# qdrant/quantization

Measured on AMD Instinct MI355X. Metric: scored vectors/sec, 10Mx768 u8 dot, higher is better.
Workload: dtype u8; 1 GPU; 10000000 x 768 store: f32 U[0,1) -> scalar u8 (dot); per step: encode_query + score_all over the shard; quantizer=u8, rows_per_gpu=10000000, dim=768, distance=dot, exchange=scores, gather_group=1, launch=single rank, world_size_seen=1, encode_ahead=False, total_rows=10000000, queries=16

## Files before the change

quantization_amd/csrc/common.hpp:

```cpp
#pragma once

#include <hip/hip_runtime.h>

#include <algorithm>
#include <atomic>
#include <mutex>
#include <cstdarg>
#include <cstdint>
#include <cstdlib>
#include <cstdio>
#include <cstring>
#include <string>
#include <vector>

#include "json.hpp"

#include "../../include/quantization_amd.h"

namespace qamd {

std::string &last_error();
qamd_status fail(qamd_status st, const char *fmt, ...) __attribute__((format(printf, 2, 3)));

#define QAMD_HIP(expr)                                                                      \
// ... 35 lines not shown
    return getenv(name);
#else
    (void)name;
    return nullptr;
#endif
}
inline uint64_t dev_env_u64(const char *name, uint64_t dflt) {
    const char *e = dev_env(name);
    if (!e || !*e) return dflt;
    char *end = nullptr;
    const unsigned long long v = strtoull(e, &end, 10);
    return (*end == 0 && v > 0) ? (uint64_t)v : dflt;
}
inline uint64_t stage_bytes(uint64_t dflt) {
    static const uint64_t v = dev_env_u64("QAMD_DEV_STAGE_BYTES", 0);
    return v ? v : dflt;
}
inline bool host_whole_allowed() {
    static const bool on = [] { const char *e = dev_env("QAMD_DEV_HOST_WHOLE"); return !(e && e[0] == '0'); }();
    return on;
}
inline bool u8_packed_allowed() {
    static const bool on = [] { const char *e = dev_env("QAMD_DEV_U8_PACKED"); return !(e && e[0] == '0'); }();
    return on;
}
inline uint64_t pq_planar_max_rows() {
    static const uint64_t v = dev_env_u64("QAMD_DEV_PQ_PLANAR_ROWS", 1ull << 28);
    return v;
}
inline uint64_t pq_skew_max_rows() {
    static const uint64_t v = dev_env_u64("QAMD_DEV_PQ_SKEW_ROWS", 1ull << 30);
    return v;
}

class DeviceOnce {
  public:
    template <class F> qamd_status run(F &&setup) {
        int dev = 0;
        if (hipGetDevice(&dev) != hipSuccess || dev < 0 || dev > 63) return setup();
        const uint64_t bit = 1ull << dev;
        if (done_.load(std::memory_order_acquire) & bit) return QAMD_OK;
        std::lock_guard<std::mutex> g(mu_);
        if (done_.load(std::memory_order_relaxed) & bit) return QAMD_OK;
        const qamd_status st = setup();
        if (st == QAMD_OK) done_.fetch_or(bit, std::memory_order_release);
        return st;
// ... 137 lines not shown
```

quantization_amd/csrc/u8.hip:

```cpp
#include <algorithm>
#include <cmath>
#include <cstdlib>
#include <memory>
#include <type_traits>
#include <vector>

#include "common.hpp"
#include "lists.hpp"
#include "multi_reduce.hpp"
#include "topk.hpp"
#include "topk_device.hpp"
#include "rescore.hpp"
#include "u8_internal.hpp"

#pragma clang fp contract(off)

using namespace qamd;

namespace {

constexpr int kBlock = 256;
constexpr int kScanBlock = 512;
constexpr uint64_t kRowPad = 1024;
constexpr uint64_t kQuantileSample = 100000;
// ... 149 lines not shown
        uint32_t acc = 0;
#pragma unroll
        for (int it = 0; it < ITERS; it++) acc = IS_L1 ? sad16(v[u][it], q[it], acc) : dot16(v[u][it], q[it], acc);
        acc = group_sum<G>(acc);
        if (sub == (u % G)) mine = epilogue(multiplier, acc, q_off, v_off[u / G], 0.0f, EPI_POINT);
        if ((u % G) == G - 1 || u == UNROLL - 1) {
            constexpr int dummy = 0;
            (void)dummy;
            const int first = (u / G) * G;
            const uint64_t row = base + (uint64_t)(first + sub) * RW + rslot;
            if (sub <= u - first && row < n_rows) {
                if (FILTER) topk_offer(filt, pivot, mine, (uint32_t)row);
                else __builtin_nontemporal_store(mine, out + row);
            }
        }
    }
}

constexpr uint32_t kPackBlockRows = 64;
constexpr uint32_t kPackBlockChunk = kPackBlockRows;

__device__ __forceinline__ uint4 and16(const uint4 &v, uint32_t m) { return make_uint4(v.x & m, v.y & m, v.z & m, v.w & m); }

template <bool FILTER>
__global__ __launch_bounds__(kScanBlock) __attribute__((amdgpu_waves_per_eu(8, 8))) void u8_scan_blocked_kernel(
    const uint4 *__restrict__ image, const float *__restrict__ offsets, const uint4 *__restrict__ qcodes,
    const float *__restrict__ q_off_p, float multiplier, uint32_t n_rows, uint32_t pchunks, uint32_t n_extra,
    uint32_t split, float *__restrict__ out, TopkFilter filt) {
    __shared__ uint32_t partial[kScanBlock];
    const uint32_t lane = threadIdx.x & 63;
    const uint32_t wave = __builtin_amdgcn_readfirstlane(threadIdx.x >> 6);
    const uint32_t part = wave & (split - 1);
    const uint64_t block = (uint64_t)blockIdx.x * ((kScanBlock / 64) / split) + wave / split;
    const uint64_t row = block * kPackBlockRows + lane;
    const bool live = block * kPackBlockRows < n_rows;
    const uint32_t n_rest = pchunks - 7 * n_extra, n_groups = n_extra + (n_rest ? 1 : 0);
    const uint32_t g_begin = live ? n_groups * part / split : 0, g_end = live ? n_groups * (part + 1) / split : 0;
    const uint4 *blk = image + block * pchunks * kPackBlockChunk;
    const uint32_t lane16 = lane * 16;
    auto chunk_ptr = [&](uint32_t c) {
        return reinterpret_cast<const uint4 *>(reinterpret_cast<const char *>(blk + (uint64_t)c * kPackBlockChunk) + lane16);
    };
    const uint32_t gf_end = g_end < n_extra ? g_end : n_extra;
    const bool has_rest = g_end > n_extra;

    uint4 v[7];
    uint32_t acc = 0;
    auto eat = [&](uint32_t g, auto refill) {
        const uint4 *q = qcodes + 7 * g;
        const uint4 qx = qcodes[pchunks + g];
#pragma unroll
        for (int i = 0; i < 7; i++) {
            const uint4 w = v[i];
            acc = dot16(and16(w, 0x7F7F7F7Fu), q[i], acc) + (dot16(and16(w, 0x80808080u), qx, 0) >> (7 - i));
            if (decltype(refill)::value) {
                __builtin_amdgcn_sched_barrier(0);
                v[i] = ld_nt(chunk_ptr(7 * (g + 1) + i));
                __builtin_amdgcn_sched_barrier(0);
            }
        }
    };
    if (g_begin < gf_end) {
#pragma unroll
        for (int i = 0; i < 7; i++) v[i] = ld_nt(chunk_ptr(7 * g_begin + i));
    }
    const float v_off = offsets[row];
    const float q_off = *q_off_p;
    uint32_t pivot = 0;
    if (FILTER) pivot = *filt.pivot_key;
    if (g_begin < gf_end) {
        for (uint32_t g = g_begin; g + 1 < gf_end; g++) eat(g, std::true_type{});
        eat(gf_end - 1, std::false_type{});
    }
    if (has_rest) {
        const uint4 *q = qcodes + 7 * n_extra;
#pragma unroll
        for (int i = 0; i < 7; i++)
            if ((uint32_t)i < n_rest) v[i] = ld_nt(chunk_ptr(7 * n_extra + i));
#pragma unroll
        for (int i = 0; i < 7; i++)
            if ((uint32_t)i < n_rest) acc = dot16(and16(v[i], 0x7F7F7F7Fu), q[i], acc);
    }
    if (split > 1) {
        partial[threadIdx.x] = acc;
        __syncthreads();
        if (part == 0)
            for (uint32_t p = 1; p < split; p++) acc += partial[threadIdx.x + 64 * p];
    }
    if (part == 0 && row < n_rows) {
        const float score = epilogue(multiplier, acc, q_off, v_off, 0.0f, EPI_POINT);
        if (FILTER) topk_offer(filt, pivot, score, (uint32_t)row);
        else __builtin_nontemporal_store(score, out + row);
    }
}

template <int G, int ITERS, int UNROLL, int NQ, bool IS_L1, bool EXACT, bool FILTER>
__global__ __launch_bounds__(kScanBlock) void u8_scan_multi_kernel(
    const uint4 *__restrict__ codes, const float *__restrict__ offsets, const uint8_t *__restrict__ qcodes,
    uint32_t q_pitch, const float *__restrict__ q_offs, uint32_t nq_valid ,
    float multiplier, uint32_t n_rows, uint32_t row_chunks, float *__restrict__ out ,
    uint64_t out_pitch, TopkFilterSlices slices) {
    static_assert(G >= NQ, "one lane of the row group per query");
    constexpr int RW = 64 / G;
    constexpr int TILE = RW * UNROLL;
    constexpr int TPW = NQ;
    const int lane = threadIdx.x & 63;
    const int sub = lane % G, rslot = lane / G;
    const uint64_t wave = ((uint64_t)blockIdx.x * kScanBlock + threadIdx.x) >> 6;
    if (wave * TILE * TPW >= n_rows) return;
    uint4 q[NQ][ITERS];
#pragma unroll
    for (int j = 0; j < NQ; j++) {
        const uint4 *qj = reinterpret_cast<const uint4 *>(qcodes + (size_t)((uint32_t)j < nq_valid ? j : nq_valid - 1) * q_pitch);
#pragma unroll
        for (int it = 0; it < ITERS; it++) {
// ... 782 lines not shown
            else QAMD_U8_GO(false, false);
        }
#undef QAMD_U8_GO
    }
};

uint32_t blocked_split(uint64_t count) {
    const uint64_t blocks = (count + kPackBlockRows - 1) / kPackBlockRows;
    const uint64_t want = (uint64_t)device_info().cu_count * 16;
    uint32_t split = 1;
    while (split < 8 && blocks * split < want) split *= 2;
    return split;
}

void launch_scan_blocked(const qamd_u8 *h, const uint4 *qc, const float *qo, float *out, const TopkFilter *filt,
                         hipStream_t s) {
    const uint32_t split = blocked_split(h->count), blocks_per_wg = (kScanBlock / 64) / split;
    const uint64_t blocks = (h->count + kPackBlockRows - 1) / kPackBlockRows;
    const unsigned grid = (unsigned)((blocks + blocks_per_wg - 1) / blocks_per_wg);
    h->last_scan_split.store((int)split, std::memory_order_relaxed);
#define QAMD_U8_BLOCKED(FI)                                                                                          \
    hipLaunchKernelGGL((u8_scan_blocked_kernel<FI>), dim3(grid), dim3(kScanBlock), 0, s, h->packed.as<uint4>(),       \
                       h->offsets.as<float>(), qc, qo, h->meta.multiplier, (uint32_t)h->count, h->packed_chunks,      \
                       h->row_chunks - h->packed_chunks, split, out, filt ? *filt : TopkFilter{})
    if (filt) QAMD_U8_BLOCKED(true);
    else QAMD_U8_BLOCKED(false);
#undef QAMD_U8_BLOCKED
}

template <bool IS_L1>
bool launch_scan(const qamd_u8 *h, const uint4 *qc, const float *qo, float *out, const TopkFilter *filt,
                 hipStream_t s) {
    using L = ScanLaunch<IS_L1>;
    const bool packed = !IS_L1 && h->packed_chunks != 0;
    h->last_scan_packed.store(packed ? 1 : 0, std::memory_order_relaxed);
    if (packed) return launch_scan_blocked(h, qc, qo, out, filt, s), true;
    const uint32_t rc = h->row_chunks;
    if (rc == 1) return L::template go<1, 1, 4>(h, qc, qo, out, filt, s), true;
    if (rc == 2) return L::template go<2, 1, 4>(h, qc, qo, out, filt, s), true;
    if (rc <= 4) return L::template go<4, 1, 8>(h, qc, qo, out, filt, s), true;
    if (rc <= 8) return L::template go<8, 1, 8>(h, qc, qo, out, filt, s), true;
    switch ((rc + 15) / 16) {
        case 1: return L::template go<16, 1, 8>(h, qc, qo, out, filt, s), true;
        case 2: return L::template go<16, 2, 4>(h, qc, qo, out, filt, s), true;
        case 3: return L::template go<16, 3, 4>(h, qc, qo, out, filt, s), true;
        case 4: return L::template go<16, 4, 2>(h, qc, qo, out, filt, s), true;
        case 5: return L::template go<16, 5, 2>(h, qc, qo, out, filt, s), true;
        case 6: return L::template go<16, 6, 2>(h, qc, qo, out, filt, s), true;
        case 7: return L::template go<16, 7, 2>(h, qc, qo, out, filt, s), true;
        case 8: return L::template go<16, 8, 2>(h, qc, qo, out, filt, s), true;
// ... 90 lines not shown
    } else {
        if (exact) QAMD_U8_MULTI(true, false);
        else QAMD_U8_MULTI(false, false);
    }
#undef QAMD_U8_MULTI
}

bool lane_order(const qamd_u8 *h) {
    return h->lane_mode == 1 && h->meta.vector_parameters.distance_type != QAMD_L1;
}

uint32_t multi_width(const qamd_u8 *h) {
    const uint32_t rc = h->row_chunks, iters = (rc + 15) / 16;
    const bool l1 = h->meta.vector_parameters.distance_type == QAMD_L1;
    if (rc < 9 || iters > 8 || lane_order(h)) return 0;
    return l1 && iters <= 3 ? 8 : iters <= 6 ? 4 : 2;
}

template <bool IS_L1>
bool launch_multi(const qamd_u8 *h, uint32_t nq_valid, const uint8_t *qcodes, uint64_t q_pitch, const float *q_offs,
                  float *out, const TopkFilterSlices *slices, hipStream_t s) {
    const uint32_t iters = (h->row_chunks + 15) / 16, width = multi_width(h);
    if (nq_valid < 2 || nq_valid > width) return false;
#define QAMD_U8_MULTI_IT(IT, UN)                                                                              \
    case IT:                                                                                                  \
        if constexpr (IS_L1 && IT <= 3) {                                                                     \
            if (nq_valid > 4) {                                                                               \
                launch_multi_shape<IS_L1, 16, IT, UN, 8>(h, qcodes, q_pitch, q_offs, nq_valid, out, slices, s); \
                return true;                                                                                  \
            }                                                                                                 \
        }                                                                                                     \
        if (nq_valid > 2) launch_multi_shape<IS_L1, 16, IT, UN, (IT <= 6 ? 4 : 2)>(h, qcodes, q_pitch, q_offs, nq_valid, out, slices, s); \
        else launch_multi_shape<IS_L1, 16, IT, UN, 2>(h, qcodes, q_pitch, q_offs, nq_valid, out, slices, s);  \
        return true;
    switch (iters) {
        QAMD_U8_MULTI_IT(1, 4) QAMD_U8_MULTI_IT(2, 2) QAMD_U8_MULTI_IT(3, 2) QAMD_U8_MULTI_IT(4, 2)
        QAMD_U8_MULTI_IT(5, 1) QAMD_U8_MULTI_IT(6, 1) QAMD_U8_MULTI_IT(7, 1) QAMD_U8_MULTI_IT(8, 1)
        default: break;
    }
#undef QAMD_U8_MULTI_IT
    return false;
}

bool fused_capable(const qamd_u8 *h) { return !lane_order(h) && h->row_chunks <= 128; }

bool u8_small_plan(const qamd_u8 *h, uint32_t k, SmallTopkPlan &plan) {
// ... 1112 lines not shown
```

quantization_amd/csrc/u8_batch.hip:

```cpp
#include <algorithm>
#include <cmath>
#include <cstdlib>
#include <memory>
#include <mutex>
#include <type_traits>
#include <vector>

#include "common.hpp"
#include "topk.hpp"
#include "topk_device.hpp"
#include "rescore.hpp"
#include "u8_internal.hpp"
#include "batch_common.hpp"
#include "u8_gemm_route.hpp"

#pragma clang fp contract(off)

using namespace qamd;

namespace {

constexpr int TQ = 256;
#ifdef QAMD_DEV
__device__ unsigned long long *g_gemm_stamps = nullptr;
// ... 486 lines not shown
                            }
                        }
                    }
                }
            }
        }
        if (ti < 3) stamp(4 + 3 * (int)ti);
        if (g == 1 && ti + 1 < my_tiles) PP_BARRIER();
    }
    stamp(15);
    if (stamps) stamps[14] = dbg_flagged;
    if (stamps) stamps[13] = __builtin_amdgcn_s_getreg((31 << 11) | 4);
    if (MODE != 0 && lane == 0) filt.wave_counts[filt.wave_base + blockIdx.x * 8 + wave] = *wcount_s;
}

template <int MI> struct RsShape {
    static constexpr int MJ = 2;
    static constexpr int TQ = 32 * MI;
    static constexpr int CHUNK = 32 * MJ;
    static constexpr int TR = 8 * CHUNK;
    static constexpr int KB = 128;
    static constexpr size_t CONSTS = 3 * 128 * sizeof(float) + 64;
    static constexpr size_t SLOTS = 8 * 4096;
    static size_t lds_bytes(uint32_t ad) { return (size_t)TQ * (round_up((uint64_t)ad, KB) + 16) + CONSTS + SLOTS; }
};

template <int MODE, bool LOW, int MI, bool NT>
__global__ __launch_bounds__(512) void u8_gemm_rs_kernel(const uint8_t *__restrict__ codes,
                                                        const float *__restrict__ v_offsets,
                                                        const uint8_t *__restrict__ qcodes, uint32_t q_pitch,
                                                        const float *__restrict__ q_offsets, float multiplier,
                                                        uint32_t n_rows, uint32_t n_queries, uint32_t ad,
                                                        uint32_t q_tiles, uint32_t row_lanes,
                                                        float *__restrict__ out, uint64_t out_pitch,
                                                        BatchFilter filt) {
    extern __shared__ __attribute__((aligned(1024))) uint8_t lds_raw[];
    using Shape = RsShape<MI>;
    constexpr int MJ = Shape::MJ, TQ = Shape::TQ, CHUNK = Shape::CHUNK, TR = Shape::TR, KB = Shape::KB;
    const int t = threadIdx.x, lane = t & 63;
    const int wave = __builtin_amdgcn_readfirstlane(t >> 6);
    const int r = lane & 31, h = lane >> 5;
    const uint32_t b = blockIdx.x, xcd = b & 7u, j = b >> 3;
    if (j >= row_lanes * q_tiles) return;
    const uint32_t q_tile = j % q_tiles, row_lane = j / q_tiles;
    const uint32_t q0 = q_tile * TQ;
    const uint32_t nkb = __builtin_amdgcn_readfirstlane((ad + KB - 1) / KB);
    const uint32_t PA = nkb * KB + 16;
    const uint32_t n_rtiles = (n_rows + TR - 1) / TR;
    const uint32_t first = xcd + 8 * row_lane, step = 8 * row_lanes;
    const uint32_t my_tiles =
        __builtin_amdgcn_readfirstlane(first < n_rtiles ? (n_rtiles - first + step - 1) / step : 0u);

    float *q_off_s = reinterpret_cast<float *>(lds_raw + (size_t)TQ * PA);
    float *pivot_s = q_off_s + 128;
    int *bq_s = reinterpret_cast<int *>(pivot_s + 128);
    uint32_t *wcount_s = reinterpret_cast<uint32_t *>(bq_s + 128) + wave;
    constexpr bool LARGEST = MODE == 1;
    if (MODE != 0 && lane == 0) *wcount_s = 0;
    if (t < TQ) {
        const float qo = q_offsets[q0 + t];
        q_off_s[t] = qo;
        if (MODE != 0) {
            const float pv = filt.pivot_scores[q0 + t];
            pivot_s[t] = pv;
            bq_s[t] = pp_query_bound<LOW>(pv, qo, multiplier, q0 + t < n_queries);
        }
    }
    {
        const uint32_t per_row = nkb * (KB / 16);
        for (uint32_t idx = t; idx < (uint32_t)TQ * per_row; idx += 512) {
            const uint32_t row = idx / per_row, k = (idx % per_row) * 16;
            v4i v = {0, 0, 0, 0};
            if (k < q_pitch) v = *reinterpret_cast<const v4i *>(qcodes + (uint64_t)(q0 + row) * q_pitch + k);
            *reinterpret_cast<v4i *>(lds_raw + row * PA + k) = v;
        }
    }
    __syncthreads();
    if (my_tiles == 0) {
        if (MODE != 0 && lane == 0) filt.wave_counts[filt.wave_base + blockIdx.x * 8 + wave] = 0;
        return;
    }

    const uint64_t row_bytes = ad;
    const uint32_t l8 = (uint32_t)lane & 7u, lrow = (uint32_t)lane >> 3;
    const uint8_t *pf0 = codes + ((uint64_t)first * TR + wave * CHUNK + lrow) * row_bytes + 16 * l8;
    const uint64_t i_stride = (uint64_t)8 * row_bytes;
    const uint64_t wrap_advance = (uint64_t)step * TR * row_bytes - (uint64_t)nkb * KB;
    uint32_t pf_kb = 0, pf_left = my_tiles * nkb - 1;
    v4i L[8];
    auto prefetch = [&]() {
        if (NT) {
#pragma unroll
            for (int i = 0; i < 8; i++) L[i] = __builtin_nontemporal_load(reinterpret_cast<const v4i *>(pf0 + i * i_stride));
        } else {
#pragma unroll
            for (int i = 0; i < 8; i++) L[i] = *reinterpret_cast<const v4i *>(pf0 + i * i_stride);
        }
        uint64_t adv = KB;
        if (++pf_kb == nkb) {
            pf_kb = 0;
            adv += wrap_advance;
        }
        if (pf_left == 0) {
            adv = 0;
            pf_kb = 0;
        } else {
            pf_left--;
        }
        pf0 += adv;
    };
    uint8_t *slot = lds_raw + (size_t)TQ * PA + Shape::CONSTS + (size_t)wave * 4096;
    uint8_t *wr = slot + lrow * 128 + ((l8 ^ (lrow & 7u)) * 16);
    const uint32_t rbase = (uint32_t)r * 128u + (((4u * (uint32_t)h) ^ ((uint32_t)r & 4u)) * 16u);
    const uint8_t *rd = slot + rbase;
    const uint32_t r3 = (uint32_t)r & 3u;
    v4i F[MJ][4];
    auto transpose = [&]() {
#pragma unroll
        for (int jj = 0; jj < MJ; jj++) {
#pragma unroll
            for (int i = 0; i < 4; i++) *reinterpret_cast<v4i *>(wr + 1024 * i) = L[4 * jj + i];
#pragma unroll
            for (int x = 0; x < 4; x++) F[jj][x] = *reinterpret_cast<const v4i *>(rd + 16u * ((uint32_t)x ^ r3));
        }
    };
    const uint8_t *a_base = lds_raw + r * PA + 64 * h;

    prefetch();
    float vo_next[MJ];
    if (MODE != 0) {
#pragma unroll
        for (int jj = 0; jj < MJ; jj++) vo_next[jj] = v_offsets[(uint64_t)first * TR + wave * CHUNK + jj * 32 + r];
    }
    const float never = LARGEST ? -__builtin_huge_valf() : __builtin_huge_valf();
    uint32_t tile = first;
    for (uint32_t ti = 0; ti < my_tiles; ti++, tile += step) {
        v16i acc[MI][MJ];
        float vo_cur[MJ];
        int br[MJ];
        const uint64_t row_a = (uint64_t)tile * TR + wave * CHUNK + r;
#pragma unroll
        for (int jj = 0; jj < MJ; jj++) {
            vo_cur[jj] = 0.0f;
            br[jj] = 0;
        }
        if (MODE == 0) {
// ... 7 lines not shown
#pragma unroll
            for (int jj = 0; jj < MJ; jj++) vo_cur[jj] = vo_next[jj];
            {
                const uint32_t nt = ti + 1 < my_tiles ? tile + step : tile;
#pragma unroll
                for (int jj = 0; jj < MJ; jj++) vo_next[jj] = v_offsets[(uint64_t)nt * TR + wave * CHUNK + jj * 32 + r];
            }
#pragma unroll
            for (int jj = 0; jj < MJ; jj++)
                br[jj] = row_a + 32 * jj < n_rows ? pp_row_bound<LOW>(vo_cur[jj], multiplier)
                                                  : (LOW ? -(int)kPpLim : (int)kPpLim);
#pragma unroll
            for (int i = 0; i < MI; i++)
#pragma unroll
                for (int gq = 0; gq < 4; gq++) {
                    const v4i bq4 = *reinterpret_cast<const v4i *>(bq_s + i * 32 + 8 * gq + 4 * h);
#pragma unroll
                    for (int e = 0; e < 4; e++)
#pragma unroll
                        for (int jj = 0; jj < MJ; jj++) acc[i][jj][4 * gq + e] = -(bq4[e] + br[jj]);
                }
        }
        for (uint32_t kb = 0; kb < nkb; kb++) {
            transpose();
            prefetch();
            const uint8_t *pa = a_base + kb * KB;
#pragma unroll
            for (int x = 0; x < 4; x++) {
                v4i a[MI];
#pragma unroll
                for (int i = 0; i < MI; i++) a[i] = *reinterpret_cast<const v4i *>(pa + (uint32_t)i * 32u * PA + 16 * x);
#pragma unroll
                for (int i = 0; i < MI; i++)
#pragma unroll
                    for (int jj = 0; jj < MJ; jj++)
                        acc[i][jj] = __builtin_amdgcn_mfma_i32_32x32x32_i8(a[i], F[jj][x], acc[i][jj], 0, 0, 0);
            }
        }

        const uint64_t row0 = (uint64_t)tile * TR + wave * CHUNK;
        uint32_t q0_e = q0, wave_e = (uint32_t)wave, lane_e = (uint32_t)lane;
        asm volatile("" : "+s"(q0_e), "+s"(wave_e), "+v"(lane_e));
        uint4 *wave_list = MODE != 0 ? filt.wave_cand + (uint64_t)(filt.wave_base + blockIdx.x * 8 + wave_e) * filt.wave_cap : nullptr;
        const uint32_t r_e = lane_e & 31u, h_e = lane_e >> 5;
#pragma unroll
        for (int jj = 0; jj < MJ; jj++) {
            const uint64_t row = row0 + jj * 32 + r_e;
// ... 978 lines not shown
    U8GemmInputs in;
    in.actual_dim = h->meta.actual_dim;
    in.rows = h->count;
    in.multiplier = h->meta.multiplier;
    in.n_queries = b->n_queries;
    in.q_pad = b->q_pad;
    in.frag_nkb = b->frag.ptr ? b->frag_nkb : 0;
    in.cu_count = device_info().cu_count;
    in.pass = pass;
    in.whole_store = n_rows == h->count;
    return u8_gemm_route(in, dev_switches().route);
}

struct GemmCall {
    const qamd_u8 *h;
    const qamd_u8_query_batch *b;
    const uint8_t *codes;
    const float *v_offsets;
    uint64_t n_rows;
    float *out;
    uint64_t out_pitch;
    BatchFilter filt;
    hipStream_t s;
};

template <int MODE, typename Fn>
qamd_status with_low(float multiplier, Fn &&fn) {
    if constexpr (MODE == 1 || MODE == 2) {
        if ((multiplier < 0.0f) != (MODE == 2)) return fn(std::true_type{});
    }
    return fn(std::false_type{});
}

template <bool LOW>
qamd_status launch_qs_bounds(const GemmCall &c) {
    hipLaunchKernelGGL(qs_bounds_kernel<LOW>, dim3((unsigned)(c.b->q_pad / 256)), dim3(256), 0, c.s, c.filt.pivot_scores,
                       c.b->offsets.as<float>(), c.h->meta.multiplier, (uint32_t)c.b->n_queries, (uint32_t)c.b->q_pad, c.filt.query_bounds);
    QAMD_HIP(hipGetLastError());
    return QAMD_OK;
}

template <int MODE, int TQ_, int TR_, int WQ, int WR, int BK_>
qamd_status launch_gemm_cfg(const GemmCall &c) {
    const uint32_t q_tiles = (uint32_t)((c.b->n_queries + TQ_ - 1) / TQ_);
    const uint64_t r_tiles = round_up((c.n_rows + TR_ - 1) / TR_, 8);
    const uint64_t blocks = r_tiles * q_tiles;
// ... 17 lines not shown
    for (uint64_t qt0 = 0; qt0 < all_q_tiles; qt0 += cus_per_xcd) {
        const uint32_t q_tiles = (uint32_t)std::min<uint64_t>(cus_per_xcd, all_q_tiles - qt0);
        const uint32_t row_lanes = cus_per_xcd / q_tiles;
        const uint64_t q_base = qt0 * TQW;
        BatchFilter f = c.filt;
        if (MODE != 0) {
            f.pivot_scores += q_base;
            f.query_base = (uint32_t)q_base;
            f.wave_base = (uint32_t)(qt0 / cus_per_xcd) * pp_waves_per_launch();
        }
        hipLaunchKernelGGL(KERNEL, dim3(8 * row_lanes * q_tiles), dim3(512), lds_bytes, c.s, c.codes, c.v_offsets,
                           b->codes.as<uint8_t>() + q_base * b->pitch, (uint32_t)b->pitch, b->offsets.as<float>() + q_base,
                           c.h->meta.multiplier, (uint32_t)c.n_rows, (uint32_t)(b->n_queries - q_base),
                           (uint32_t)c.h->meta.actual_dim, q_tiles, row_lanes, MODE == 0 ? c.out + q_base * c.out_pitch : c.out,
                           c.out_pitch, f);
        QAMD_HIP(hipGetLastError());
    }
    return QAMD_OK;
}
template <int MODE, bool LOW, int MI, int MJ>
qamd_status launch_gemm_pp(const GemmCall &c) {
    return launch_tile_sliced<MODE, &u8_gemm_pp_kernel<MODE, LOW, MI, MJ>, 64 * MI, (int)PpShape<MI, MJ>::LDS>(c, PpShape<MI, MJ>::LDS);
}
template <int MODE, bool LOW, int MI, bool NT>
qamd_status launch_gemm_rs(const GemmCall &c) {
    return launch_tile_sliced<MODE, &u8_gemm_rs_kernel<MODE, LOW, MI, NT>, 32 * MI, 160 * 1024>(
        c, RsShape<MI>::lds_bytes((uint32_t)c.h->meta.actual_dim));
}

template <int MODE, typename LaunchSlice>
qamd_status launch_query_sliced(const GemmCall &c, uint64_t slice, LaunchSlice &&launch_slice) {
    for (uint64_t q_base = 0; q_base < c.b->n_queries; q_base += slice) {
        const uint32_t nq = (uint32_t)std::min<uint64_t>(slice, c.b->n_queries - q_base);
        BatchFilter f = c.filt;
        if (MODE == 1 || MODE == 2) {
            f.pivot_scores += q_base;
            f.query_base = (uint32_t)q_base;
            f.wave_base = (uint32_t)(q_base / slice) * pp_waves_per_launch();
        }
        launch_slice(q_base, nq, f);
        QAMD_HIP(hipGetLastError());
    }
    return QAMD_OK;
}
template <int MODE, bool LOW, int JT, int IT>
qamd_status launch_gemm_qs16(const GemmCall &c) {
    QAMD_LDS_OPT_IN((&u8_gemm_qs16_kernel<MODE, LOW, JT, IT>), 160 * 1024);
    constexpr bool FILTER = MODE == 1 || MODE == 2;
    constexpr int QS_ROWS = 16 * JT;
    const qamd_u8_query_batch *b = c.b;
// ... 75 lines not shown
                }
                break;
            case K::Rq16:
                if constexpr (FILTER) {
                    switch (rt.nsteps) {
                        case 4: return launch_gemm_rq<MODE, LOW, 4, 0>(c, rt.rq);
                        case 6: return launch_gemm_rq<MODE, LOW, 6, 0>(c, rt.rq);
                        case 8: return launch_gemm_rq<MODE, LOW, 8, 0>(c, rt.rq);
                        case 12: return launch_gemm_rq<MODE, LOW, 12, 0>(c, rt.rq);
                    }
                }
                break;
            case K::Rk16:
                if constexpr (FILTER) {
                    switch (rt.nt_tiles) {
                        case 8: return launch_gemm_rq<MODE, LOW, 12, 8>(c, rt.rq);
                        case 10: return launch_gemm_rq<MODE, LOW, 12, 10>(c, rt.rq);
                        case 12: return launch_gemm_rq<MODE, LOW, 12, 12>(c, rt.rq);
                    }
                }
                break;
            case K::Rs:
                if constexpr (MODE != 3) {
                    switch (rt.mi * 2 + (rt.nt ? 1 : 0)) {
                        case 9: return launch_gemm_rs<MODE, LOW, 4, true>(c);
                        case 8: return launch_gemm_rs<MODE, LOW, 4, false>(c);
                        case 5: return launch_gemm_rs<MODE, LOW, 2, true>(c);
                        case 4: return launch_gemm_rs<MODE, LOW, 2, false>(c);
                        case 3: return launch_gemm_rs<MODE, LOW, 1, true>(c);
                        case 2: return launch_gemm_rs<MODE, LOW, 1, false>(c);
                    }
                }
                break;
            case K::Pp:
                if constexpr (MODE != 3) {
                    if (rt.mi == 2 && rt.mj == 4) return launch_gemm_pp<MODE, LOW, 2, 4>(c);
                    if (rt.mi == 4 && rt.mj == 2) return launch_gemm_pp<MODE, LOW, 4, 2>(c);
                }
                break;
            case K::Gemm:
                if constexpr (MODE != 3) {
                    if (rt.tile == 128) return launch_gemm_cfg<MODE, 128, 128, 2, 2, 128>(c);
                    if (rt.tile == 256) return launch_gemm_cfg<MODE, 256, 256, 2, 4, 128>(c);
                }
                break;
        }
// ... 1 lines not shown
    });
}

qamd_status sample_store(const qamd_u8 *h, uint32_t rows_all, hipStream_t s, const uint8_t **codes, const float **offs) {
    std::lock_guard<std::mutex> lk(h->sample_mu);
    if (h->sample_rows < rows_all) {
        const uint64_t ad = h->meta.actual_dim;
        qamd::DevBuf c, o;
        QAMD_TRY(c.alloc((uint64_t)(rows_all + 512) * ad));
        QAMD_TRY(o.alloc((uint64_t)(rows_all + 512) * 4));
        hipLaunchKernelGGL(gather_rows_kernel, dim3(device_info().cu_count * 8), dim3(256), 0, s, h->codes.as<uint4>(),
                           h->offsets.as<float>(), h->row_chunks, h->count, rows_all, 512u, c.as<uint4>(), o.as<float>());
        QAMD_HIP(hipGetLastError());
        QAMD_HIP(hipStreamSynchronize(s));
        h->sample_codes = std::move(c);
        h->sample_offsets = std::move(o);
        h->sample_rows = rows_all;
    }
    *codes = h->sample_codes.as<uint8_t>();
    *offs = h->sample_offsets.as<float>();
    return QAMD_OK;
}

}

extern "C" {

#ifdef QAMD_GEMM_ABLATION
QAMD_API qamd_status qamd_dev_gemm_debug(unsigned int flags) {
    QAMD_HIP(hipMemcpyToSymbol(HIP_SYMBOL(g_gemm_dbg), &flags, sizeof(flags)));
    return QAMD_OK;
}
#endif

#ifdef QAMD_DEV
QAMD_API qamd_status qamd_dev_gemm_stamps(void *dev_buffer) {
    QAMD_HIP(hipMemcpyToSymbol(HIP_SYMBOL(g_gemm_stamps), &dev_buffer, sizeof(void *)));
    return QAMD_OK;
}
#endif

qamd_status qamd_u8_encode_query_batch(const qamd_u8 *h, const float *queries, uint64_t n_queries, uint64_t qdim,
                                       qamd_mem queries_mem, void *stream, qamd_u8_query_batch **batch_io) {
    if (!h || !batch_io || (!queries && n_queries && qdim)) return fail(QAMD_ERR_ARGUMENTS, "null argument");
    QAMD_ON_DEVICE(h->device);
    hipStream_t s = as_stream(stream);
    const uint64_t ad = qdim + (16 - qdim % 16) % 16;
    qamd_u8_query_batch *b = *batch_io;
    std::unique_ptr<qamd_u8_query_batch> fresh;
    if (!b) {
        fresh.reset(new qamd_u8_query_batch);
        b = fresh.get();
        b->device = h->device;
    }
    const uint64_t q_pad = round_up(std::max<uint64_t>(n_queries, 1), TQ);
    const uint64_t pitch = round_up(std::max<uint64_t>(ad, 16), 64);
    if (b->actual_dim != ad || b->q_pad != q_pad || !b->codes.ptr) {
        b->pitch = pitch;
        QAMD_TRY(b->codes.alloc(q_pad * pitch, true));
        QAMD_TRY(b->offsets.alloc(q_pad * sizeof(float), true));
        b->actual_dim = ad;
        b->q_pad = q_pad;
// ... 39 lines not shown
    QAMD_ON_DEVICE(h->device);
    hipStream_t s = as_stream(stream);
    return run_lists(list_offsets, n_lists, ids, n_ids, nullptr, lists_mem, out, out_mem, h->count, s, [&](const ListArgs &a) {
        return u8_score_lists(h, b->codes.as<uint8_t>(), b->pitch, b->offsets.as<float>(), a, s);
    });
}

qamd_status qamd_u8_score_batch(const qamd_u8 *h, const qamd_u8_query_batch *b, float *out, qamd_mem out_mem,
                                void *stream) {
    QAMD_TRY(check_batch(h, b));
    if (h->count == 0 || b->n_queries == 0) return QAMD_OK;
    if (!out) return fail(QAMD_ERR_ARGUMENTS, "out is null");
    QAMD_ON_DEVICE(h->device);
    hipStream_t s = as_stream(stream);
    const uint64_t total = b->n_queries * h->count;
    DevBuf tmp;
    float *out_dev = out;
    if (out_mem == QAMD_MEM_HOST) {
        QAMD_TRY(tmp.alloc(total * 4));
        out_dev = tmp.as<float>();
    }
    const uint32_t width = u8_multi_width(h);
    const U8GemmRoute route = gemm_route(h, b, U8GemmPass::Score, h->count);
    if (h->meta.vector_parameters.distance_type == QAMD_L1 || u8_lane_order(h) ||
        (width && b->n_queries >= 2 && b->n_queries <= width && (b->n_queries == 2 || !route.rs_ok))) {
        QAMD_TRY(u8_score_batch_scans(h, b->codes.as<uint8_t>(), b->pitch, b->offsets.as<float>(), (uint32_t)b->n_queries,
                                      out_dev, s));
    } else {
        QAMD_TRY(launch_gemm<0>(route, {h, b, h->codes.as<uint8_t>(), h->offsets.as<float>(), h->count, out_dev, h->count,
                                        BatchFilter{}, s}));
    }
    if (out_mem == QAMD_MEM_HOST) QAMD_TRY(copy_out(out, QAMD_MEM_HOST, out_dev, total * 4, s));
    return QAMD_OK;
}

qamd_status qamd_u8_topk_batch(const qamd_u8 *h, const qamd_u8_query_batch *b, uint32_t k, int largest,
                               uint32_t *out_ids, float *out_scores, qamd_mem out_mem, void *stream) {
    QAMD_TRY(check_batch(h, b));
    qamd_status args = QAMD_OK;
    if (!topk_wanted(k, b->n_queries, out_ids, out_scores, args)) return args;
    QAMD_ON_DEVICE(h->device);
    hipStream_t s = as_stream(stream);
    const uint64_t Q = b->n_queries, n = h->count;
    const bool l1 = h->meta.vector_parameters.distance_type == QAMD_L1;
    if (u8_lane_order(h))
        return u8_topk_batch_scans(h, b->codes.as<uint8_t>(), b->pitch, b->offsets.as<float>(), (uint32_t)Q, k, largest,
                                   out_ids, out_scores, out_mem, s);
    const U8GemmRoute filter_route = gemm_route(h, b, U8GemmPass::Filter, n);
    if (n > (2u << 20) && (l1 || (Q <= u8_multi_width(h) && Q >= 2 && (Q == 2 || !filter_route.rs_ok))))
        return u8_topk_batch_scans(h, b->codes.as<uint8_t>(), b->pitch, b->offsets.as<float>(), (uint32_t)Q, k, largest,
                                   out_ids, out_scores, out_mem, s);
    const double want = std::max<double>(Q <= 128 ? 1024.0 : 512.0, 3.0 * k);
    const double s_min = n < (1u << 20) ? 2048.0 : (double)kTopkSample;
    const double s_mem_cap = std::max<double>(s_min, std::floor((double)(6ull << 30) / (4.0 * (double)Q) / 256.0) * 256.0);
    const uint32_t S = (uint32_t)std::min<double>(std::min<double>(524288.0, s_mem_cap),
                                                  std::max<double>(s_min, round_up((uint64_t)(8.0 * (double)n / want), 256)));
    const double target = std::max<double>(want, 8.0 * (double)n / (double)S);
    const uint32_t r = n ? (uint32_t)std::ceil((double)S * target / (double)n) : 0;
    const bool fused = n >= 32768 && r <= 64 && h->meta.vector_parameters.distance_type != QAMD_L1;

    StreamBuf ids_tmp, sc_tmp;
    uint32_t *ids_dev = out_ids;
    float *sc_dev = out_scores;
    if (out_mem == QAMD_MEM_HOST) {
        QAMD_TRY(ids_tmp.alloc(Q * k * 4, s));
        QAMD_TRY(sc_tmp.alloc(Q * k * 4, s));
        ids_dev = ids_tmp.as<uint32_t>();
// ... 59 lines not shown
            const uint32_t s_blocks = (S + rows_per_block - 1) / rows_per_block;
            BatchFilter fs{};
            fs.largest = largest;
            QAMD_TRY(launch_gemm<3>(sample_route, {h, b, s_codes, s_offs, S, s_scores, s_blocks, fs, s}));
            hipLaunchKernelGGL(batch_pivot_kernel, dim3((unsigned)b->q_pad), dim3(1024), 0, s, s_scores, s_blocks,
                               (uint64_t)s_blocks, r, largest, (uint32_t)Q, pivots, counters);
        } else {
            QAMD_TRY(launch_gemm<0>(sample_route, {h, b, s_codes, s_offs, S, s_scores, S, BatchFilter{}, s}));
            hipLaunchKernelGGL(batch_pivot_kernel, dim3((unsigned)b->q_pad), dim3(1024), 0, s, s_scores, S, (uint64_t)S, r,
                               largest, (uint32_t)Q, pivots, counters);
        }
        BatchFilter f{};
        f.pivot_scores = pivots;
        f.counters = counters;
        f.candidates = cand;
        f.largest = largest;
        f.n_queries = (uint32_t)Q;
        f.query_bounds = reinterpret_cast<int *>(base + o_bounds);
        if (pp) {
            f.wave_cap = wave_cap;
            f.wave_cand = wave_cand;
            f.wave_counts = wave_counts;
        }
        if (largest)
            QAMD_TRY(launch_gemm<1>(filter_route, {h, b, h->codes.as<uint8_t>(), h->offsets.as<float>(), n, nullptr, 0, f, s}));
        else
            QAMD_TRY(launch_gemm<2>(filter_route, {h, b, h->codes.as<uint8_t>(), h->offsets.as<float>(), n, nullptr, 0, f, s}));
        if (pp && Q <= 4096)
            hipLaunchKernelGGL(wave_scatter_grouped_kernel, dim3(std::min<uint32_t>(n_lists, 128)), dim3(1024), (size_t)Q * 8, s,
                               wave_cand, wave_counts, f.wave_cap, n_lists, (uint32_t)Q, counters, cand, overflow_dev);
        else if (pp)
            hipLaunchKernelGGL(wave_scatter_kernel, dim3(n_lists), dim3(256), 0, s, wave_cand, wave_counts, f.wave_cap,
                               counters, cand, overflow_dev);
        if (k <= kSmallTopkMaxK)
            hipLaunchKernelGGL(batch_emit_wave_kernel, dim3((unsigned)Q), dim3(1024), 0, s, cand, counters, n, k, largest,
                               ids_dev, sc_dev, status_dev);
        else
            hipLaunchKernelGGL(batch_emit_kernel, dim3((unsigned)Q), dim3(1024), 0, s, cand, counters, n, k, largest, ids_dev,
                               sc_dev, status_dev);
        QAMD_HIP(hipGetLastError());
        uint32_t overflow = 0;
        if (hs.host) {
            QAMD_HIP(hipStreamSynchronize(s));
            std::copy(hs.host, hs.host + Q, status.begin());
            overflow = hs.host[Q];
        } else {
            std::vector<uint32_t> back(Q + 1);
            QAMD_TRY(copy_out(back.data(), QAMD_MEM_HOST, status_dev, (Q + 1) * 4, s));
            std::copy(back.begin(), back.begin() + Q, status.begin());
            overflow = back[Q];
// ... 48 lines not shown
```

quantization_amd/csrc/u8_internal.hpp:

```cpp
#pragma once
#include <atomic>
#include <mutex>

#include "common.hpp"
#include "lists.hpp"

struct qamd_u8 {
    int device = 0;
    qamd_u8_metadata meta{};
    uint64_t count = 0;
    uint64_t padded_rows = 0;
    uint32_t row_chunks = 0;
    int lane_mode = 0;
    qamd::DevBuf codes;
    qamd::DevBuf offsets;
    qamd::DevBuf packed;
    uint32_t packed_chunks = 0;
    mutable std::atomic<int> last_scan_packed{0};
    mutable std::atomic<int> last_scan_split{0};
    mutable qamd::DevBuf packed_rows;
    mutable std::mutex sample_mu;
    mutable qamd::DevBuf sample_codes, sample_offsets;
    mutable uint32_t sample_rows = 0;
};

struct qamd_u8_query {
    int device = 0;
    uint64_t actual_dim = 0;
    qamd::DevBuf buf;
    mutable qamd::ReadyEvent ready;
    mutable std::vector<float> host_f32;
    float alpha = 0.0f, offset = 0.0f;
    int distance = 0, invert = 0;
    mutable std::atomic<bool> deferred{false};
    mutable std::mutex encode_mu;
    bool pooled = false;
    mutable std::atomic<bool> async_used{false};
    ~qamd_u8_query() {
        if (pooled) qamd::query_buf_put(buf, !async_used.load(std::memory_order_relaxed) && ready.complete());
    }
};
// ... 37 lines not shown
```

Baseline: 9.952 billion vectors/s.

## Stream packed 7/8-byte blocked image in batch u8 scoring paths

Batch scoring now reads the packed blocked image, which stores seven low-7-bit chunks plus one shared high-bit chunk per group, instead of the full u8 codes. A two-query variant of the blocked scan kernel handles the nq=2 case. The register-staged GEMM kernel unpacks blocks in registers with permlane32 swaps instead of doing an LDS transpose, and remaps query chunk order to match. This cuts code bytes streamed from HBM by about one eighth, at the cost of extra unpack ALU work and more complex indexing.

Result: no change. 9.955 billion vectors/s (median of 4 runs) (+0.0%).

```diff
diff --git a/quantization_amd/csrc/common.hpp b/quantization_amd/csrc/common.hpp
--- a/quantization_amd/csrc/common.hpp
+++ b/quantization_amd/csrc/common.hpp
@@ -81,6 +81,10 @@
 }
 inline bool u8_packed_allowed() {
     static const bool on = [] { const char *e = dev_env("QAMD_DEV_U8_PACKED"); return !(e && e[0] == '0'); }();
+    return on;
+}
+inline bool u8_batch_packed_allowed() {
+    static const bool on = [] { const char *e = dev_env("QAMD_DEV_U8_BATCH_PACKED"); return !(e && e[0] == '0'); }();
     return on;
 }
 inline uint64_t pq_planar_max_rows() {
diff --git a/quantization_amd/csrc/u8.hip b/quantization_amd/csrc/u8.hip
--- a/quantization_amd/csrc/u8.hip
+++ b/quantization_amd/csrc/u8.hip
@@ -195,12 +195,13 @@
 
 __device__ __forceinline__ uint4 and16(const uint4 &v, uint32_t m) { return make_uint4(v.x & m, v.y & m, v.z & m, v.w & m); }
 
-template <bool FILTER>
+template <bool FILTER, int NQ = 1>
 __global__ __launch_bounds__(kScanBlock) __attribute__((amdgpu_waves_per_eu(8, 8))) void u8_scan_blocked_kernel(
     const uint4 *__restrict__ image, const float *__restrict__ offsets, const uint4 *__restrict__ qcodes,
     const float *__restrict__ q_off_p, float multiplier, uint32_t n_rows, uint32_t pchunks, uint32_t n_extra,
-    uint32_t split, float *__restrict__ out, TopkFilter filt) {
-    __shared__ uint32_t partial[kScanBlock];
+    uint32_t split, float *__restrict__ out, TopkFilter filt, uint32_t q_pitch16 = 0, uint64_t out_pitch = 0,
+    TopkFilterSlices slices = TopkFilterSlices{}) {
+    __shared__ uint32_t partial[NQ][kScanBlock];
     const uint32_t lane = threadIdx.x & 63;
     const uint32_t wave = __builtin_amdgcn_readfirstlane(threadIdx.x >> 6);
     const uint32_t part = wave & (split - 1);
@@ -218,14 +219,25 @@
     const bool has_rest = g_end > n_extra;
 
     uint4 v[7];
-    uint32_t acc = 0;
+    uint32_t acc[NQ];
+#pragma unroll
+    for (int j = 0; j < NQ; j++) acc[j] = 0;
     auto eat = [&](uint32_t g, auto refill) {
         const uint4 *q = qcodes + 7 * g;
-        const uint4 qx = qcodes[pchunks + g];
+        uint4 qx[NQ];
+#pragma unroll
+        for (int j = 0; j < NQ; j++) qx[j] = qcodes[(size_t)j * q_pitch16 + pchunks + g];
 #pragma unroll
         for (int i = 0; i < 7; i++) {
             const uint4 w = v[i];
-            acc = dot16(and16(w, 0x7F7F7F7Fu), q[i], acc) + (dot16(and16(w, 0x80808080u), qx, 0) >> (7 - i));
+            if constexpr (NQ == 1) {
+                acc[0] = dot16(and16(w, 0x7F7F7F7Fu), q[i], acc[0]) + (dot16(and16(w, 0x80808080u), qx[0], 0) >> (7 - i));
+            } else {
+                const uint4 lo = and16(w, 0x7F7F7F7Fu), hi = and16(w, 0x80808080u);
+#pragma unroll
+                for (int j = 0; j < NQ; j++)
+                    acc[j] = dot16(lo, q[(size_t)j * q_pitch16 + i], acc[j]) + (dot16(hi, qx[j], 0) >> (7 - i));
+            }
             if (decltype(refill)::value) {
                 __builtin_amdgcn_sched_barrier(0);
                 v[i] = ld_nt(chunk_ptr(7 * (g + 1) + i));
@@ -238,32 +250,50 @@
         for (int i = 0; i < 7; i++) v[i] = ld_nt(chunk_ptr(7 * g_begin + i));
     }
     const float v_off = offsets[row];
-    const float q_off = *q_off_p;
+    float q_off[NQ];
+#pragma unroll
+    for (int j = 0; j < NQ; j++) q_off[j] = q_off_p[j];
     uint32_t pivot = 0;
-    if (FILTER) pivot = *filt.pivot_key;
+    if (FILTER && NQ == 1) pivot = *filt.pivot_key;
     if (g_begin < gf_end) {
         for (uint32_t g = g_begin; g + 1 < gf_end; g++) eat(g, std::true_type{});
         eat(gf_end - 1, std::false_type{});
     }
     if (has_rest) {
-        const uint4 *q = qcodes + 7 * n_extra;
 #pragma unroll
         for (int i = 0; i < 7; i++)
             if ((uint32_t)i < n_rest) v[i] = ld_nt(chunk_ptr(7 * n_extra + i));
 #pragma unroll
         for (int i = 0; i < 7; i++)
-            if ((uint32_t)i < n_rest) acc = dot16(and16(v[i], 0x7F7F7F7Fu), q[i], acc);
+            if ((uint32_t)i < n_rest) {
+                const uint4 lo = and16(v[i], 0x7F7F7F7Fu);
+#pragma unroll
+                for (int j = 0; j < NQ; j++) acc[j] = dot16(lo, (qcodes + (size_t)j * q_pitch16)[7 * n_extra + i], acc[j]);
+            }
     }
     if (split > 1) {
-        partial[threadIdx.x] = acc;
+#pragma unroll
+        for (int j = 0; j < NQ; j++) partial[j][threadIdx.x] = acc[j];
         __syncthreads();
         if (part == 0)
-            for (uint32_t p = 1; p < split; p++) acc += partial[threadIdx.x + 64 * p];
+            for (uint32_t p = 1; p < split; p++)
+#pragma unroll
+                for (int j = 0; j < NQ; j++) acc[j] += partial[j][threadIdx.x + 64 * p];
     }
     if (part == 0 && row < n_rows) {
-        const float score = epilogue(multiplier, acc, q_off, v_off, 0.0f, EPI_POINT);
-        if (FILTER) topk_offer(filt, pivot, score, (uint32_t)row);
-        else __builtin_nontemporal_store(score, out + row);
+#pragma unroll
+        for (int j = 0; j < NQ; j++) {
+            const float score = epilogue(multiplier, acc[j], q_off[j], v_off, 0.0f, EPI_POINT);
+            if constexpr (NQ == 1) {
+                if (FILTER) topk_offer(filt, pivot, score, (uint32_t)row);
+                else __builtin_nontemporal_store(score, out + row);
+            } else if (FILTER) {
+                const TopkFilter f = topk_filter_of(slices, (uint32_t)j);
+                topk_offer(f, *f.pivot_key, score, (uint32_t)row);
+            } else {
+                __builtin_nontemporal_store(score, out + (uint64_t)j * out_pitch + row);
+            }
+        }
     }
 }
 
@@ -1092,10 +1122,27 @@
 #define QAMD_U8_BLOCKED(FI)                                                                                          \
     hipLaunchKernelGGL((u8_scan_blocked_kernel<FI>), dim3(grid), dim3(kScanBlock), 0, s, h->packed.as<uint4>(),       \
                        h->offsets.as<float>(), qc, qo, h->meta.multiplier, (uint32_t)h->count, h->packed_chunks,      \
-                       h->row_chunks - h->packed_chunks, split, out, filt ? *filt : TopkFilter{})
+                       h->row_chunks - h->packed_chunks, split, out, filt ? *filt : TopkFilter{}, 0u, (uint64_t)0,    \
+                       TopkFilterSlices{})
     if (filt) QAMD_U8_BLOCKED(true);
     else QAMD_U8_BLOCKED(false);
 #undef QAMD_U8_BLOCKED
+}
+
+void launch_scan_blocked2(const qamd_u8 *h, const uint8_t *qcodes, uint64_t q_pitch, const float *q_offs, float *out,
+                          const TopkFilterSlices *slices, hipStream_t s) {
+    const uint32_t split = blocked_split(h->count), blocks_per_wg = (kScanBlock / 64) / split;
+    const uint64_t blocks = (h->count + kPackBlockRows - 1) / kPackBlockRows;
+    const unsigned grid = (unsigned)((blocks + blocks_per_wg - 1) / blocks_per_wg);
+#define QAMD_U8_BLOCKED2(FI)                                                                                         \
+    hipLaunchKernelGGL((u8_scan_blocked_kernel<FI, 2>), dim3(grid), dim3(kScanBlock), 0, s, h->packed.as<uint4>(),    \
+                       h->offsets.as<float>(), reinterpret_cast<const uint4 *>(qcodes), q_offs, h->meta.multiplier,   \
+                       (uint32_t)h->count, h->packed_chunks, h->row_chunks - h->packed_chunks, split, out, TopkFilter{}, \
+                       (uint32_t)(q_pitch / 16), (uint64_t)h->count, slices ? *slices : TopkFilterSlices{})
+    if (slices) QAMD_U8_BLOCKED2(true);
+    else QAMD_U8_BLOCKED2(false);
+#undef QAMD_U8_BLOCKED2
+    h->last_batch_packed.store(1, std::memory_order_relaxed);
 }
 
 template <bool IS_L1>
@@ -1232,6 +1279,10 @@
                   float *out, const TopkFilterSlices *slices, hipStream_t s) {
     const uint32_t iters = (h->row_chunks + 15) / 16, width = multi_width(h);
     if (nq_valid < 2 || nq_valid > width) return false;
+    if constexpr (!IS_L1) {
+        if (nq_valid == 2 && h->packed_chunks != 0 && u8_batch_packed_allowed())
+            return launch_scan_blocked2(h, qcodes, q_pitch, q_offs, out, slices, s), true;
+    }
 #define QAMD_U8_MULTI_IT(IT, UN)                                                                              \
     case IT:                                                                                                  \
         if constexpr (IS_L1 && IT <= 3) {                                                                     \
diff --git a/quantization_amd/csrc/u8_batch.hip b/quantization_amd/csrc/u8_batch.hip
--- a/quantization_amd/csrc/u8_batch.hip
+++ b/quantization_amd/csrc/u8_batch.hip
@@ -532,10 +532,10 @@
     static constexpr int KB = 128;
     static constexpr size_t CONSTS = 3 * 128 * sizeof(float) + 64;
     static constexpr size_t SLOTS = 8 * 4096;
-    static size_t lds_bytes(uint32_t ad) { return (size_t)TQ * (round_up((uint64_t)ad, KB) + 16) + CONSTS + SLOTS; }
+    static size_t lds_bytes(uint32_t ad, bool blk) { return (size_t)TQ * (round_up((uint64_t)ad, KB) + 16) + CONSTS + (blk ? 0 : SLOTS); }
 };
 
-template <int MODE, bool LOW, int MI, bool NT>
+template <int MODE, bool LOW, int MI, bool NT, bool BLK = false>
 __global__ __launch_bounds__(512) void u8_gemm_rs_kernel(const uint8_t *__restrict__ codes,
                                                         const float *__restrict__ v_offsets,
                                                         const uint8_t *__restrict__ qcodes, uint32_t q_pitch,
@@ -576,13 +576,20 @@
             bq_s[t] = pp_query_bound<LOW>(pv, qo, multiplier, q0 + t < n_queries);
         }
     }
+    const uint32_t rc = ad / 16, n_extra = rc / 8, n_rest = rc % 8, P = rc - n_extra;
     {
         const uint32_t per_row = nkb * (KB / 16);
         for (uint32_t idx = t; idx < (uint32_t)TQ * per_row; idx += 512) {
-            const uint32_t row = idx / per_row, k = (idx % per_row) * 16;
+            const uint32_t row = idx / per_row, slot_i = idx % per_row;
+            uint32_t k = slot_i * 16;
+            if (BLK) {
+                const uint32_t g = slot_i / 8, i = slot_i % 8;
+                const uint32_t c = g < n_extra ? (i < 7 ? 7 * g + i : P + g) : (i < n_rest ? 7 * n_extra + i : rc);
+                k = c < rc ? c * 16 : q_pitch;
+            }
             v4i v = {0, 0, 0, 0};
             if (k < q_pitch) v = *reinterpret_cast<const v4i *>(qcodes + (uint64_t)(q0 + row) * q_pitch + k);
-            *reinterpret_cast<v4i *>(lds_raw + row * PA + k) = v;
+            *reinterpret_cast<v4i *>(lds_raw + row * PA + slot_i * 16) = v;
         }
     }
     __syncthreads();
@@ -591,29 +598,40 @@
         return;
     }
 
-    const uint64_t row_bytes = ad;
+    const uint64_t row_bytes = BLK ? (uint64_t)P * 16 : ad;
     const uint32_t l8 = (uint32_t)lane & 7u, lrow = (uint32_t)lane >> 3;
-    const uint8_t *pf0 = codes + ((uint64_t)first * TR + wave * CHUNK + lrow) * row_bytes + 16 * l8;
-    const uint64_t i_stride = (uint64_t)8 * row_bytes;
-    const uint64_t wrap_advance = (uint64_t)step * TR * row_bytes - (uint64_t)nkb * KB;
+    constexpr uint64_t kStreamStep = BLK ? 7 * 1024 : KB;
+    const uint8_t *pf0 = BLK ? codes + (uint64_t)(first * 8 + wave) * row_bytes * 64 + 16 * lane
+                             : codes + ((uint64_t)first * TR + wave * CHUNK + lrow) * row_bytes + 16 * l8;
+    const uint64_t i_stride = BLK ? 1024 : (uint64_t)8 * row_bytes;
+    const uint64_t wrap_advance = (uint64_t)step * TR * row_bytes - (uint64_t)nkb * kStreamStep;
     uint32_t pf_kb = 0, pf_left = my_tiles * nkb - 1;
     v4i L[8];
     auto prefetch = [&]() {
-        if (NT) {
+        if (BLK) {
+            if (pf_kb < n_extra) {
+#pragma unroll
+                for (int i = 0; i < 7; i++) L[i] = __builtin_nontemporal_load(reinterpret_cast<const v4i *>(pf0 + i * i_stride));
+            } else {
+#pragma unroll
+                for (int i = 0; i < 7; i++)
+                    if ((uint32_t)i < n_rest) L[i] = __builtin_nontemporal_load(reinterpret_cast<const v4i *>(pf0 + i * i_stride));
+            }
+        } else if (NT) {
 #pragma unroll
             for (int i = 0; i < 8; i++) L[i] = __builtin_nontemporal_load(reinterpret_cast<const v4i *>(pf0 + i * i_stride));
         } else {
 #pragma unroll
             for (int i = 0; i < 8; i++) L[i] = *reinterpret_cast<const v4i *>(pf0 + i * i_stride);
         }
-        uint64_t adv = KB;
+        uint64_t adv = kStreamStep;
         if (++pf_kb == nkb) {
             pf_kb = 0;
             adv += wrap_advance;
         }
         if (pf_left == 0) {
             adv = 0;
-            pf_kb = 0;
+            pf_kb = nkb - 1;
         } else {
             pf_left--;
         }
@@ -625,13 +643,46 @@
     const uint8_t *rd = slot + rbase;
     const uint32_t r3 = (uint32_t)r & 3u;
     v4i F[MJ][4];
-    auto transpose = [&]() {
-#pragma unroll
-        for (int jj = 0; jj < MJ; jj++) {
-#pragma unroll
-            for (int i = 0; i < 4; i++) *reinterpret_cast<v4i *>(wr + 1024 * i) = L[4 * jj + i];
-#pragma unroll
-            for (int x = 0; x < 4; x++) F[jj][x] = *reinterpret_cast<const v4i *>(rd + 16u * ((uint32_t)x ^ r3));
+    auto transpose = [&](uint32_t kb) {
+        if constexpr (BLK) {
+            static_assert(MJ == 2, "a block of the image is the wave's two 32-row fragments");
+            v4i V[8];
+            if (kb < n_extra) {
+#pragma unroll
+                for (int d = 0; d < 4; d++) {
+                    uint32_t extra = 0;
+#pragma unroll
+                    for (int i = 0; i < 7; i++) {
+                        const uint32_t w = (uint32_t)L[i][d];
+                        V[i][d] = (int)(w & 0x7F7F7F7Fu);
+                        extra |= (w & 0x80808080u) >> (7 - i);
+                    }
+                    V[7][d] = (int)extra;
+                }
+            } else {
+#pragma unroll
+                for (int i = 0; i < 7; i++)
+#pragma unroll
+                    for (int d = 0; d < 4; d++) V[i][d] = (uint32_t)i < n_rest ? (int)((uint32_t)L[i][d] & 0x7F7F7F7Fu) : 0;
+#pragma unroll
+                for (int d = 0; d < 4; d++) V[7][d] = 0;
+            }
+#pragma unroll
+            for (int x = 0; x < 4; x++)
+#pragma unroll
+                for (int d = 0; d < 4; d++) {
+                    const auto sw = __builtin_amdgcn_permlane32_swap((uint32_t)V[x][d], (uint32_t)V[4 + x][d], false, false);
+                    F[0][x][d] = (int)sw[0];
+                    F[1][x][d] = (int)sw[1];
+                }
+        } else {
+#pragma unroll
+            for (int jj = 0; jj < MJ; jj++) {
+#pragma unroll
+                for (int i = 0; i < 4; i++) *reinterpret_cast<v4i *>(wr + 1024 * i) = L[4 * jj + i];
+#pragma unroll
+                for (int x = 0; x < 4; x++) F[jj][x] = *reinterpret_cast<const v4i *>(rd + 16u * ((uint32_t)x ^ r3));
+            }
         }
     };
     const uint8_t *a_base = lds_raw + r * PA + 64 * h;
@@ -685,7 +736,7 @@
                 }
         }
         for (uint32_t kb = 0; kb < nkb; kb++) {
-            transpose();
+            transpose(kb);
             prefetch();
             const uint8_t *pa = a_base + kb * KB;
 #pragma unroll
@@ -1710,6 +1761,7 @@
     uint64_t out_pitch;
     BatchFilter filt;
     hipStream_t s;
+    bool blocked = false;
 };
 
 template <int MODE, typename Fn>
@@ -1773,10 +1825,10 @@
 qamd_status launch_gemm_pp(const GemmCall &c) {
     return launch_tile_sliced<MODE, &u8_gemm_pp_kernel<MODE, LOW, MI, MJ>, 64 * MI, (int)PpShape<MI, MJ>::LDS>(c, PpShape<MI, MJ>::LDS);
 }
-template <int MODE, bool LOW, int MI, bool NT>
+template <int MODE, bool LOW, int MI, bool NT, bool BLK = false>
 qamd_status launch_gemm_rs(const GemmCall &c) {
-    return launch_tile_sliced<MODE, &u8_gemm_rs_kernel<MODE, LOW, MI, NT>, 32 * MI, 160 * 1024>(
-        c, RsShape<MI>::lds_bytes((uint32_t)c.h->meta.actual_dim));
+    return launch_tile_sliced<MODE, &u8_gemm_rs_kernel<MODE, LOW, MI, NT, BLK>, 32 * MI, 160 * 1024>(
+        c, RsShape<MI>::lds_bytes((uint32_t)c.h->meta.actual_dim, BLK));
 }
 
 template <int MODE, typename LaunchSlice>
@@ -1898,6 +1950,14 @@
                 break;
             case K::Rs:
                 if constexpr (MODE != 3) {
+                    if (c.blocked) {
+                        switch (rt.nt ? rt.mi : 0) {
+                            case 4: return launch_gemm_rs<MODE, LOW, 4, true, true>(c);
+                            case 2: return launch_gemm_rs<MODE, LOW, 2, true, true>(c);
+                            case 1: return launch_gemm_rs<MODE, LOW, 1, true, true>(c);
+                        }
+                        break;
+                    }
                     switch (rt.mi * 2 + (rt.nt ? 1 : 0)) {
                         case 9: return launch_gemm_rs<MODE, LOW, 4, true>(c);
                         case 8: return launch_gemm_rs<MODE, LOW, 4, false>(c);
@@ -1945,6 +2005,13 @@
     return QAMD_OK;
 }
 
+bool batch_blocked(const qamd_u8 *h, const U8GemmRoute &rt) {
+    const bool blocked = rt.kernel == U8GemmKernel::Rs && rt.nt && h->packed_chunks != 0 && u8_batch_packed_allowed();
+    if (blocked) h->last_batch_packed.store(1, std::memory_order_relaxed);
+    return blocked;
+}
+const uint8_t *batch_rows(const qamd_u8 *h, bool blocked) { return blocked ? h->packed.as<uint8_t>() : h->codes.as<uint8_t>(); }
+
 }
 
 extern "C" {
@@ -1961,6 +2028,7 @@
     QAMD_HIP(hipMemcpyToSymbol(HIP_SYMBOL(g_gemm_stamps), &dev_buffer, sizeof(void *)));
     return QAMD_OK;
 }
+QAMD_API int qamd_dev_u8_last_batch_packed(const qamd_u8 *h) { return h->last_batch_packed.load(std::memory_order_relaxed); }
 #endif
 
 qamd_status qamd_u8_encode_query_batch(const qamd_u8 *h, const float *queries, uint64_t n_queries, uint64_t qdim,
@@ -2046,13 +2114,15 @@
     }
     const uint32_t width = u8_multi_width(h);
     const U8GemmRoute route = gemm_route(h, b, U8GemmPass::Score, h->count);
+    h->last_batch_packed.store(0, std::memory_order_relaxed);
     if (h->meta.vector_parameters.distance_type == QAMD_L1 || u8_lane_order(h) ||
         (width && b->n_queries >= 2 && b->n_queries <= width && (b->n_queries == 2 || !route.rs_ok))) {
         QAMD_TRY(u8_score_batch_scans(h, b->codes.as<uint8_t>(), b->pitch, b->offsets.as<float>(), (uint32_t)b->n_queries,
                                       out_dev, s));
     } else {
-        QAMD_TRY(launch_gemm<0>(route, {h, b, h->codes.as<uint8_t>(), h->offsets.as<float>(), h->count, out_dev, h->count,
-                                        BatchFilter{}, s}));
+        const bool blocked = batch_blocked(h, route);
+        QAMD_TRY(launch_gemm<0>(route, {h, b, batch_rows(h, blocked), h->offsets.as<float>(), h->count, out_dev, h->count,
+                                        BatchFilter{}, s, blocked}));
     }
     if (out_mem == QAMD_MEM_HOST) QAMD_TRY(copy_out(out, QAMD_MEM_HOST, out_dev, total * 4, s));
     return QAMD_OK;
@@ -2067,6 +2137,7 @@
     hipStream_t s = as_stream(stream);
     const uint64_t Q = b->n_queries, n = h->count;
     const bool l1 = h->meta.vector_parameters.distance_type == QAMD_L1;
+    h->last_batch_packed.store(0, std::memory_order_relaxed);
     if (u8_lane_order(h))
         return u8_topk_batch_scans(h, b->codes.as<uint8_t>(), b->pitch, b->offsets.as<float>(), (uint32_t)Q, k, largest,
                                    out_ids, out_scores, out_mem, s);
@@ -2172,10 +2243,11 @@
             f.wave_cand = wave_cand;
             f.wave_counts = wave_counts;
         }
+        const bool blocked = batch_blocked(h, filter_route);
         if (largest)
-            QAMD_TRY(launch_gemm<1>(filter_route, {h, b, h->codes.as<uint8_t>(), h->offsets.as<float>(), n, nullptr, 0, f, s}));
+            QAMD_TRY(launch_gemm<1>(filter_route, {h, b, batch_rows(h, blocked), h->offsets.as<float>(), n, nullptr, 0, f, s, blocked}));
         else
-            QAMD_TRY(launch_gemm<2>(filter_route, {h, b, h->codes.as<uint8_t>(), h->offsets.as<float>(), n, nullptr, 0, f, s}));
+            QAMD_TRY(launch_gemm<2>(filter_route, {h, b, batch_rows(h, blocked), h->offsets.as<float>(), n, nullptr, 0, f, s, blocked}));
         if (pp && Q <= 4096)
             hipLaunchKernelGGL(wave_scatter_grouped_kernel, dim3(std::min<uint32_t>(n_lists, 128)), dim3(1024), (size_t)Q * 8, s,
                                wave_cand, wave_counts, f.wave_cap, n_lists, (uint32_t)Q, counters, cand, overflow_dev);
diff --git a/quantization_amd/csrc/u8_internal.hpp b/quantization_amd/csrc/u8_internal.hpp
--- a/quantization_amd/csrc/u8_internal.hpp
+++ b/quantization_amd/csrc/u8_internal.hpp
@@ -17,6 +17,7 @@
     qamd::DevBuf packed;
     uint32_t packed_chunks = 0;
     mutable std::atomic<int> last_scan_packed{0};
+    mutable std::atomic<int> last_batch_packed{0};
     mutable std::atomic<int> last_scan_split{0};
     mutable qamd::DevBuf packed_rows;
     mutable std::mutex sample_mu;
```
